# vadimkantorov/deepspeech.pytorch

Hardware: AMD Instinct MI355X
Metric: audio-seconds/sec training, DS2 5x BiGRU-800 bs32, at 1/2/4/8 MI355X (higher is better)
Workload: dtype f32

## Files before the change

### deepspeech.pytorch_amd/csrc/gru_xl.hip

```cpp
#include "rnn_host.h"

#include <algorithm>

namespace ds2 {

#ifndef DS2_XL_ABL
#define DS2_XL_ABL 0
#endif
constexpr bool kAblLoads = (DS2_XL_ABL & 1) != 0;
constexpr bool kAblStores = (DS2_XL_ABL & 2) != 0;
constexpr bool kAblWait = (DS2_XL_ABL & 4) != 0;
constexpr bool kAblFixT = (DS2_XL_ABL & 8) != 0;

constexpr int LB = 8;
constexpr int LU = 32;
constexpr int LW = 4;
constexpr int LT = LW * 64;
constexpr int LSLOTS = 4;
constexpr int LRB = 784;
constexpr int kXlTraceS0 = 100, kXlTraceSteps = 16;

__device__ __forceinline__ bool xl_map(int G, int UBX, int& g, int& ub) {
  g = blockIdx.x & 7;
  ub = blockIdx.x >> 3;
  return g < G && ub < UBX;
}

__device__ __forceinline__ bool xl_group_local(unsigned* xtab, int ub, int UBX, unsigned* err,
                                               unsigned* err_out, int* lds_word, unsigned* mode,
                                               int force_global) {
  const unsigned mine = xcc_id() + 1u;
  if (threadIdx.x == 0) __hip_atomic_store(xtab + ub, mine, __ATOMIC_RELAXED, __HIP_MEMORY_SCOPE_AGENT);
  if ((threadIdx.x >> 6) == 0) {
    const int lane = threadIdx.x & 63;
    unsigned v = mine;
    bool ok = true;
    for (unsigned spins = 0;; ++spins) {
      v = lane < UBX ? __hip_atomic_load(xtab + lane, __ATOMIC_RELAXED, __HIP_MEMORY_SCOPE_AGENT)
                     : mine;
      if (__ballot(v == 0u) == 0ull) break;
      if (spins > g_spin_limit) {
        if (lane == 0) raise_err(err, err_out);
        ok = false;
        break;
      }
      __builtin_amdgcn_s_sleep(1);
    }
    const bool loc = ok && __ballot(v != mine) == 0ull && force_global == 0;
    if (lane == 0) {
      *lds_word = loc ? 1 : 0;
      __hip_atomic_fetch_or(mode, loc ? 1u : 2u, __ATOMIC_RELAXED, __HIP_MEMORY_SCOPE_AGENT);
    }
  }
  __syncthreads();
  return *lds_word != 0;
}

__device__ __forceinline__ void xl_store(u32x4 v, __amdgpu_buffer_rsrc_t rs, int off, bool local) {
  if (local)
    __builtin_amdgcn_raw_buffer_store_b128(v, rs, off, 0, 0);
  else
    __builtin_amdgcn_raw_buffer_store_b128(v, rs, off, 0, kSc1);
}

#define DS2_DPP_MAX(v, ctrl)                                                               \
  v = fmaxf(v, __builtin_bit_cast(float, __builtin_amdgcn_update_dpp(                      \
                   0, __builtin_bit_cast(int, v), ctrl, 0xf, 0xf, true)))
__device__ __forceinline__ float half_wave_max(float v) {
  DS2_DPP_MAX(v, 0xB1);
  DS2_DPP_MAX(v, 0x4E);
  DS2_DPP_MAX(v, 0x141);
  DS2_DPP_MAX(v, 0x140);
  const int b = __builtin_bit_cast(int, v);
  const float r0 = __builtin_bit_cast(float, __builtin_amdgcn_readlane(b, 0));
  const float r1 = __builtin_bit_cast(float, __builtin_amdgcn_readlane(b, 16));
  const float r2 = __builtin_bit_cast(float, __builtin_amdgcn_readlane(b, 32));
  const float r3 = __builtin_bit_cast(float, __builtin_amdgcn_readlane(b, 48));
  return (threadIdx.x & 32) ? fmaxf(r2, r3) : fmaxf(r0, r1);
}
#undef DS2_DPP_MAX

__device__ __forceinline__ bool xl_wave_flags_wait(const unsigned* flags, int count,
                                                   unsigned target, unsigned* err,
                                                   unsigned* err_out) {
  const int lane = threadIdx.x & 63;
  if (count == 0) return true;
  for (unsigned spins = 0;; ++spins) {
    if (spins > g_spin_limit || g_spin_limit == 0) {
      if (lane == 0) raise_err(err, err_out);
      return false;
    }
    const unsigned v = lane < count ? __hip_atomic_load(flags + lane, __ATOMIC_RELAXED,
                                                        __HIP_MEMORY_SCOPE_AGENT)
                                    : target;
    if (__ballot(v < target) == 0ull) return true;
    sleep_units(g_rnn_tune[3]);
  }
}

__device__ __forceinline__ int xl_frag_hi(int m, int k) { return (((k >> 3) << 4) + m) * 8 + (k & 7); }

template <int NPW>
__global__ __launch_bounds__(LT) __attribute__((amdgpu_waves_per_eu(1, 1))) void gru_fwd_xl_kernel(
    int T, int N, int H, int D, int UBX, int BTX, const float* __restrict__ xproj,
    const float* __restrict__ w_f, const float* __restrict__ w_r, const float* __restrict__ b_f,
    const float* __restrict__ b_r, const int* __restrict__ lens, float* __restrict__ h_all,
    float* __restrict__ gates, float* __restrict__ ring, unsigned* __restrict__ xl,
    unsigned* __restrict__ err, unsigned* __restrict__ err_out,
    unsigned long long* __restrict__ stamps, int force_global) {
  constexpr int NCT = 6;
  constexpr int RC = 3 * LU + 1;
  __shared__ float red[LW * 16 * RC];
  __shared__ __attribute__((aligned(16))) _Float16 stg[64 * 8];
  __shared__ float unsc[3 * LU];
  __shared__ __attribute__((aligned(16))) float pin[3 * 256];
  __shared__ __attribute__((aligned(16))) float pout[5 * 256];
  __shared__ int slen[LB];
  __shared__ int sh_local;
  __shared__ int failed;
  __shared__ u32x4 wx[LW * NCT * 2 * 64];
  const int G = D * BTX;
  int g, ub;
  if (!xl_map(G, UBX, g, ub)) return;
  const int d = g / BTX, bt = g - d * BTX;
  const int lane = threadIdx.x & 63;
  const int wave = __builtin_amdgcn_readfirstlane(threadIdx.x >> 6);
  const int p0 = wave * (UBX / LW) + min(wave, UBX % LW);
  const int np = UBX / LW + (wave < UBX % LW ? 1 : 0);
  if (threadIdx.x == 0) failed = 0;
  const bool local =
      xl_group_local(xl + g * 32, ub, UBX, err, err_out, &sh_local, xl + 512 + g, force_global);
  const int slot_floats = G * UBX * 256;
  const __amdgpu_buffer_rsrc_t x_rs =
      __builtin_amdgcn_make_buffer_rsrc(ring, (short)0, LSLOTS * slot_floats * 4, 0x00020000);
  const int grp_off = g * UBX * 256;
  const bool tracing = stamps != nullptr && lane == 0;
  auto trace_at = [&](int s, int p) __attribute__((always_inline)) {
    if (tracing && s >= kXlTraceS0 && s < kXlTraceS0 + kXlTraceSteps)
      stamps[(((int64_t)(s - kXlTraceS0) * gridDim.x + blockIdx.x) * LW + wave) * 6 + p] =
          __builtin_amdgcn_s_memrealtime();
  };

  Duo w[NPW][NCT];
  auto wfr = [&](int p, int ct) __attribute__((always_inline)) {
    if (p < NPW) return w[p < NPW ? p : 0][ct];
    Duo r;
    r.hi = __builtin_bit_cast(f16x8, wx[((wave * NCT + ct) * 2 + 0) * 64 + lane]);
    r.lo = __builtin_bit_cast(f16x8, wx[((wave * NCT + ct) * 2 + 1) * 64 + lane]);
    return r;
  };
  {
    const float* W = d == 0 ? w_f : w_r;
    const int q8 = 8 * (lane >> 4);
    auto frag = [&](int p, int ct, f32x4& a, f32x4& b) __attribute__((always_inline)) {
      const f32x4 z4 = f32x4{0.f, 0.f, 0.f, 0.f};
      if (p < np) {
        const float* r = W + (int64_t)((ct >> 1) * H + LU * ub + 16 * (ct & 1) + (lane & 15)) * H +
                         LU * (p0 + p) + q8;
        a = *reinterpret_cast<const f32x4*>(r);
        b = *reinterpret_cast<const f32x4*>(r + 4);
      } else {
        a = z4;
        b = z4;
      }
    };
    float mx[NCT];
#pragma unroll
    for (int ct = 0; ct < NCT; ++ct) mx[ct] = 0.f;
#pragma unroll
    for (int p = 0; p < NPW + 1; ++p)
#pragma unroll
      for (int ct = 0; ct < NCT; ++ct) {
        f32x4 a, b;
        frag(p, ct, a, b);
#pragma unroll
        for (int i = 0; i < 4; ++i) mx[ct] = fmaxf(mx[ct], fmaxf(fabsf(a[i]), fabsf(b[i])));
      }
#pragma unroll
    for (int ct = 0; ct < NCT; ++ct) {
      mx[ct] = fmaxf(mx[ct], __shfl_xor(mx[ct], 16));
      mx[ct] = fmaxf(mx[ct], __shfl_xor(mx[ct], 32));
      if (lane < 16) red[wave * 96 + ct * 16 + lane] = mx[ct];
    }
    __syncthreads();
    float sc[NCT];
#pragma unroll
    for (int ct = 0; ct < NCT; ++ct) {
      float m = 0.f;
#pragma unroll
      for (int w4 = 0; w4 < LW; ++w4) m = fmaxf(m, red[w4 * 96 + ct * 16 + (lane & 15)]);
      sc[ct] = __builtin_ldexpf(1.f, h3_row_exp(m));
    }
    if (threadIdx.x < 3 * LU) {
      float m = 0.f;
#pragma unroll
      for (int w4 = 0; w4 < LW; ++w4) m = fmaxf(m, red[w4 * 96 + threadIdx.x]);
      unsc[threadIdx.x] = __builtin_ldexpf(1.f, -(h3_row_exp(m) + 14));
    }
    __syncthreads();
    asm volatile("" ::: "memory");
#pragma unroll
    for (int p = 0; p < NPW + 1; ++p)
#pragma unroll
      for (int ct = 0; ct < NCT; ++ct) {
        f32x4 a, b;
        frag(p, ct, a, b);
        const Duo dd = split2h(a, b, sc[ct]);
        if (p < NPW) {
          w[p < NPW ? p : 0][ct] = dd;
        } else {
          wx[((wave * NCT + ct) * 2 + 0) * 64 + lane] = __builtin_bit_cast(u32x4, dd.hi);
          wx[((wave * NCT + ct) * 2 + 1) * 64 + lane] = __builtin_bit_cast(u32x4, dd.lo);
        }
      }
  }
  const float* bh = d == 0 ? b_f : b_r;
  const int m = threadIdx.x >> 5;
  const int u = threadIdx.x & 31;
  const int n = bt * LB + m;
  const int j = ub * LU + u;
  const bool owner = n < N;
  float bias_r = 0.f, bias_z = 0.f, bias_n = 0.f;
  if (owner) {
    bias_r = bh[j];
    bias_z = bh[H + j];
    bias_n = bh[2 * H + j];
  }
  if (threadIdx.x < LB) slen[threadIdx.x] = bt * LB + (int)threadIdx.x < N ? lens[bt * LB + threadIdx.x] : 0;
  __syncthreads();
  const int len = slen[m];
  const float us_r = unsc[u], us_z = unsc[LU + u], us_n = unsc[2 * LU + u];
  settle(bias_r);
  settle(bias_z);
  settle(bias_n);
  const int shi = xl_frag_hi(m, u), slo = shi + 64;
  const bool io = wave != 0;
  const int q = io ? (int)threadIdx.x - 64 : 0;
  const int qm = q / 24, qg = (q % 24) >> 3, q4 = (q & 7) * 4;
  const int qn = bt * LB + qm;
  const bool qv = io && qn < N;
  const int qlen = slen[qm];
  const float* xq = xproj + ((int64_t)qn * D + d) * 3 * H + qg * H + ub * LU + q4;
  const int64_t xstep = (int64_t)N * D * 3 * H;
  const f32x4 z4v = f32x4{0.f, 0.f, 0.f, 0.f};
  auto in_ok = [&](int st) __attribute__((always_inline)) {
    const int tt = d == 0 ? st : T - 1 - st;
    return !kAblLoads && qv && tt < qlen;
  };
  auto load_in = [&](int st) __attribute__((always_inline)) {
    const int tt = d == 0 ? st : T - 1 - st;
    return *reinterpret_cast<const f32x4*>(in_ok(st) ? xq + (kAblFixT ? 0 : tt) * xstep : xproj);
  };
  float* ob[2];
  int64_t ostr[2];
  int osrc[2];
  bool ov[2];
#pragma unroll
  for (int k = 0; k < 2; ++k) {
    const int idx = q + 192 * k;
    const int sm = (idx / 40) & 7, f = (idx % 40) >> 3, o4 = (idx & 7) * 4, sn = bt * LB + sm;
    ov[k] = io && idx < 320 && sn < N && (f == 0 || gates != nullptr);
    osrc[k] = f * 256 + sm * LU + o4;
    if (f == 0) {
      ob[k] = h_all + ((int64_t)sn * D + d) * H + ub * LU + o4;
      ostr[k] = (int64_t)N * D * H;
    } else {
      ob[k] = gates + ((int64_t)sn * D + d) * 4 * H + (f - 1) * H + ub * LU + o4;
      ostr[k] = (int64_t)N * D * 4 * H;
    }
  }
  auto store_out = [&](int st) __attribute__((always_inline)) {
    const int tt = d == 0 ? st : T - 1 - st;
#pragma unroll
    for (int k = 0; k < 2; ++k)
      if (ov[k])
        *reinterpret_cast<f32x4*>(ob[k] + tt * ostr[k]) = *reinterpret_cast<const f32x4*>(pout + osrc[k]);
  };
  f32x4 xin = io ? load_in(0) : z4v;
  float h_own = 0.f;
  for (int s = 0; s < T; ++s) {
    const int t = d == 0 ? s : T - 1 - s;
    f32x4 acc[NCT];
#pragma unroll
    for (int ct = 0; ct < NCT; ++ct) acc[ct] = f32x4{0.f, 0.f, 0.f, 0.f};
    trace_at(s, 0);
    if (io) *reinterpret_cast<f32x4*>(pin + qg * 256 + qm * LU + q4) = in_ok(s) ? xin : z4v;
    if (s > 0) {
      trace_at(s, 1);
      const int base = (((s - 1) % LSLOTS) * slot_floats + grp_off + p0 * 256 + lane * 4) * 4;
      sleep_units(g_rnn_tune[7]);
      u32x4 hv[NPW + 1];
#pragma unroll
      for (int p = 0; p < NPW + 1; ++p)
        hv[p] = __builtin_amdgcn_raw_buffer_load_b128(x_rs, p < np ? base + p * 1024 : 0x7ffffff0, 0, kSc1);
      asm volatile("" ::: "memory");
      __builtin_amdgcn_sched_barrier(0);
      bool bad = false;
#pragma unroll
      for (int p = 0; p < NPW + 1; ++p) {
        if (p < np && !bad) {
          for (unsigned spins = 0;
               !kAblWait && (!wave_ready(__builtin_bit_cast(f32x4, hv[p])) || g_spin_limit == 0);
               ++spins) {
            if (spins > g_spin_limit || g_spin_limit == 0) {
              if (lane == 0) raise_err(err, err_out);
              failed = 1;
              bad = true;
              break;
            }
            sleep_units(g_rnn_tune[0]);
            asm volatile("" ::: "memory");
#pragma unroll
            for (int q = p; q < NPW + 1; ++q)
              if (q < np && (unsigned)(q - p) < g_rnn_tune[6])
                hv[q] = __builtin_amdgcn_raw_buffer_load_b128(x_rs, base + q * 1024, 0, kSc1);
          }
          const f16x8 a = __builtin_bit_cast(f16x8, hv[p]);
#pragma unroll
          for (int ct = 0; ct < NCT; ++ct) {
            const Duo wf = wfr(p, ct);
            acc[ct] = __builtin_amdgcn_mfma_f32_16x16x32_f16(a, wf.lo, acc[ct], 0, 0, 0);
            acc[ct] = __builtin_amdgcn_mfma_f32_16x16x32_f16(a, wf.hi, acc[ct], 0, 0, 0);
          }
        }
      }
      trace_at(s, 2);
    }
    if (io) {
      if (s + 1 < T) xin = load_in(s + 1);
      if (!kAblStores && s > 0) store_out(s - 1);
    }
    trace_at(s, 3);
#pragma unroll
    for (int ct = 0; ct < NCT; ++ct)
#pragma unroll
      for (int i = 0; i < 4; ++i)
        red[(wave * 16 + (lane >> 4) * 4 + i) * RC + ct * 16 + (lane & 15)] = acc[ct][i];
    __syncthreads();
    if (failed) {
      poison_rest(h_all, s, T, d != 0, N, D, n, d, H, j, H, 1, owner);
      return;
    }
    trace_at(s, 4);
    float gh[3];
#pragma unroll
    for (int gt = 0; gt < 3; ++gt) {
      float v = 0.f;
#pragma unroll
      for (int w4 = 0; w4 < LW; ++w4)
        v += red[(w4 * 16 + m) * RC + gt * LU + u] + red[(w4 * 16 + m + 8) * RC + gt * LU + u];
      gh[gt] = v;
    }
    const float xr = pin[m * LU + u], xz = pin[256 + m * LU + u], xn = pin[512 + m * LU + u];
    float hout = 0.f, r = 0.f, z = 0.f, nn = 0.f, ghn = 0.f;
    if (owner && t < len) {
      ghn = gh[2] * us_n + bias_n;
      r = sigmoid_fast(gh[0] * us_r + bias_r + xr);
      z = sigmoid_fast(gh[1] * us_z + bias_z + xz);
      nn = tanh_fast(xn + r * ghn);
      hout = (h_own - nn) * z + nn;
    }
    h_own = owner ? hout : 0.f;
    pout[m * LU + u] = hout;
    pout[256 + m * LU + u] = r;
    pout[512 + m * LU + u] = z;
    pout[768 + m * LU + u] = nn;
    pout[1024 + m * LU + u] = ghn;
    {
      const float v = hout * 16384.f;
      const _Float16 hi = (_Float16)v;
      stg[shi] = hi;
      stg[slo] = (_Float16)(v - (float)hi);
    }
    __syncthreads();
    if (wave == 0) {
      const int toff = (grp_off + ub * 256 + lane * 4) * 4;
      const u32x4 v = desentinel(*reinterpret_cast<const u32x4*>(stg + lane * 8));
      asm volatile("s_waitcnt vmcnt(0)" ::: "memory");
      xl_store(v, x_rs, (s % LSLOTS) * slot_floats * 4 + toff, local);
      xl_store(u32x4{kSentinel, kSentinel, kSentinel, kSentinel}, x_rs,
               ((s + 2) % LSLOTS) * slot_floats * 4 + toff, local);
    }
    trace_at(s, 5);
  }
  __syncthreads();
  if (io && !kAblStores) store_out(T - 1);
}

template <int NPW, bool ROWS>
__global__ __launch_bounds__(LT) __attribute__((amdgpu_waves_per_eu(1, 1))) void gru_bwd_xl_kernel(
    int T, int N, int H, int D, int UBX, int BTX, const float* __restrict__ dy, int dyd,
    const float* __restrict__ w_f, const float* __restrict__ w_r,
    const float* __restrict__ h_all, const float* __restrict__ gates,
    const int* __restrict__ lens, float* __restrict__ dgx, float* __restrict__ dgh,
    float* __restrict__ ring, unsigned* __restrict__ xl, unsigned* __restrict__ err,
    unsigned* __restrict__ err_out, unsigned long long* __restrict__ stamps,
    double* __restrict__ dbp, unsigned* __restrict__ camax, float* __restrict__ rowp,
    int force_global) {
  constexpr int RC = LU + 1;
  constexpr int LWP = 3;
  __shared__ __attribute__((aligned(8))) float red[LW * 16 * RC > 4 * LB * LU * 2 ? LW * 16 * RC : 4 * LB * LU * 2];
  __shared__ __attribute__((aligned(16))) _Float16 stg[3 * 64 * 8];
  __shared__ __attribute__((aligned(16))) float stsc[LB];
  __shared__ float colmx[LW * LU];
  __shared__ __attribute__((aligned(16))) float pin[6 * 256];
  __shared__ __attribute__((aligned(16))) float pout[4 * 256];
  __shared__ int slen[LB];
  __shared__ int sh_local;
  __shared__ int flag;
  __shared__ float rowmx[2 * LB];
  __shared__ u32x4 wx[LW * 6 * 2 * 64];
  const int G = D * BTX;
  int g, ub;
  if (!xl_map(G, UBX, g, ub)) return;
  const int d = g / BTX, bt = g - d * BTX;
  const int lane = threadIdx.x & 63;
  const int wave = __builtin_amdgcn_readfirstlane(threadIdx.x >> 6);
  const int p0 = wave * (UBX / LW) + min(wave, UBX % LW);
  const int np = UBX / LW + (wave < UBX % LW ? 1 : 0);
  const int H3 = 3 * H;
  if (threadIdx.x == 0) flag = 1;
  const int slot_floats = G * UBX * LRB;
  const __amdgpu_buffer_rsrc_t x_rs =
      __builtin_amdgcn_make_buffer_rsrc(ring, (short)0, 2 * slot_floats * 4, 0x00020000);
  const int grp_off = g * UBX * LRB;
  const bool local =
      xl_group_local(xl + g * 32, ub, UBX, err, err_out, &sh_local, xl + 512 + g, force_global);
  unsigned* flags = xl + 256 + g * 32;
  const __amdgpu_buffer_rsrc_t f_rs =
      __builtin_amdgcn_make_buffer_rsrc(xl + 256, (short)0, 8 * 32 * 4, 0x00020000);
  const bool tracing = stamps != nullptr && lane == 0;
  auto trace_at = [&](int s, int p) __attribute__((always_inline)) {
    if (tracing && s >= kXlTraceS0 && s < kXlTraceS0 + kXlTraceSteps)
      stamps[(((int64_t)(s - kXlTraceS0) * gridDim.x + blockIdx.x) * LW + wave) * 6 + p] =
          __builtin_amdgcn_s_memrealtime();
  };

  Duo w[NPW][3][2];
  auto wfr = [&](int p, int gt, int c) __attribute__((always_inline)) {
    if (p < NPW) return w[p < NPW ? p : 0][gt][c];
    Duo r;
    r.hi = __builtin_bit_cast(f16x8, wx[((wave * 6 + gt * 2 + c) * 2 + 0) * 64 + lane]);
    r.lo = __builtin_bit_cast(f16x8, wx[((wave * 6 + gt * 2 + c) * 2 + 1) * 64 + lane]);
    return r;
  };
  float unscale;
  {
    const float* W = d == 0 ? w_f : w_r;
    const int q8 = 8 * (lane >> 4);
    auto col = [&](int p, int gt, int c, f32x4& a, f32x4& b) __attribute__((always_inline)) {
      if (p < np) {
        const float* wc = W + (int64_t)(gt * H + LU * (p0 + p) + q8) * H + LU * ub + 16 * c + (lane & 15);
#pragma unroll
        for (int i = 0; i < 4; ++i) {
          a[i] = wc[(int64_t)i * H];
          b[i] = wc[(int64_t)(i + 4) * H];
        }
      } else {
        a = f32x4{0.f, 0.f, 0.f, 0.f};
        b = a;
      }
    };
    float mx[2] = {0.f, 0.f};
#pragma unroll
    for (int p = 0; p < NPW + 1; ++p)
#pragma unroll
      for (int gt = 0; gt < 3; ++gt)
#pragma unroll
        for (int c = 0; c < 2; ++c) {
          f32x4 a, b;
          col(p, gt, c, a, b);
#pragma unroll
          for (int i = 0; i < 4; ++i) mx[c] = fmaxf(mx[c], fmaxf(fabsf(a[i]), fabsf(b[i])));
        }
#pragma unroll
    for (int c = 0; c < 2; ++c) {
      mx[c] = fmaxf(mx[c], __shfl_xor(mx[c], 16));
      mx[c] = fmaxf(mx[c], __shfl_xor(mx[c], 32));
      if (lane < 16) colmx[wave * LU + 16 * c + lane] = mx[c];
    }
    __syncthreads();
    float sc[2];
#pragma unroll
    for (int c = 0; c < 2; ++c) {
      float m = 0.f;
#pragma unroll
      for (int w4 = 0; w4 < LW; ++w4) m = fmaxf(m, colmx[w4 * LU + 16 * c + (lane & 15)]);
      sc[c] = __builtin_ldexpf(1.f, h3_row_exp(m));
    }
    {
      float m = 0.f;
#pragma unroll
      for (int w4 = 0; w4 < LW; ++w4) m = fmaxf(m, colmx[w4 * LU + (threadIdx.x & 31)]);
      unscale = __builtin_ldexpf(1.f, -h3_row_exp(m));
    }
    asm volatile("" ::: "memory");
#pragma unroll
    for (int p = 0; p < NPW + 1; ++p)
#pragma unroll
      for (int gt = 0; gt < 3; ++gt)
#pragma unroll
        for (int c = 0; c < 2; ++c) {
          f32x4 a, b;
          col(p, gt, c, a, b);
          const Duo dd = split2h(a, b, sc[c]);
          if (p < NPW) {
            w[p < NPW ? p : 0][gt][c] = dd;
          } else {
            wx[((wave * 6 + gt * 2 + c) * 2 + 0) * 64 + lane] = __builtin_bit_cast(u32x4, dd.hi);
            wx[((wave * 6 + gt * 2 + c) * 2 + 1) * 64 + lane] = __builtin_bit_cast(u32x4, dd.lo);
          }
        }
  }
  const int m = threadIdx.x >> 5;
  const int u = threadIdx.x & 31;
  const int n = bt * LB + m;
  const int j = ub * LU + u;
  const bool owner = n < N;
  if (threadIdx.x < LB) slen[threadIdx.x] = bt * LB + (int)threadIdx.x < N ? lens[bt * LB + threadIdx.x] : 0;
  __syncthreads();
  const int len = slen[m];
  const int shi = xl_frag_hi(m, u), slo = shi + 64;
  const bool io = wave != 0;
  const int q = io ? (int)threadIdx.x - 64 : 0;
  const f32x4 z4v = f32x4{0.f, 0.f, 0.f, 0.f};
  const int ostr = N * D * H3;
  struct IoSlot {
    const float* in;
    float* out;
    int f, len, str, pin_at, pout_at;
  };
  auto make_slot = [&](int k) __attribute__((always_inline)) {
    const int idx = q + 192 * k;
    const int sm = idx / 48, f = (idx % 48) >> 3, o4 = (idx & 7) * 4, sn = bt * LB + sm;
    IoSlot r;
    r.f = f;
    r.len = io && sn < N ? slen[sm] : -1;
    if (f == 0) {
      r.in = dy + (sn * dyd + (dyd > 1 ? d : 0)) * H + ub * LU + o4;
      r.str = N * dyd * H;
    } else if (f < 5) {
      r.in = gates + (sn * D + d) * 4 * H + (f - 1) * H + ub * LU + o4;
      r.str = N * D * 4 * H;
    } else {
      r.in = h_all + (sn * D + d) * H + ub * LU + o4;
      r.str = N * D * H;
    }
    r.out = io && sn < N ? (f < 3 ? dgx : dgh) + (sn * D + d) * H3 + (f % 3) * H + ub * LU + o4
                         : nullptr;
    r.pin_at = f * 256 + sm * LU + o4;
    r.pout_at = (f < 3 ? f : (f == 5 ? 3 : f - 3)) * 256 + sm * LU + o4;
    return r;
  };
  const IoSlot sl0 = make_slot(0), sl1 = make_slot(1);
  auto in_ok = [&](int st, const IoSlot sl) __attribute__((always_inline)) {
    const int tt = d == 0 ? T - 1 - st : st;
    const int tr = sl.f == 5 ? (d == 0 ? tt - 1 : tt + 1) : tt;
    return !kAblLoads && tt < sl.len && tr >= 0 && tr < T;
  };
  auto load_in = [&](int st, const IoSlot sl) __attribute__((always_inline)) {
    const int tt = d == 0 ? T - 1 - st : st;
    const int tr = sl.f == 5 ? (d == 0 ? tt - 1 : tt + 1) : tt;
    return *reinterpret_cast<const f32x4*>(sl.in + (in_ok(st, sl) && !kAblFixT ? tr * sl.str : 0));
  };
  auto stage_in = [&](const f32x4 v, const IoSlot sl, int st) __attribute__((always_inline)) {
    *reinterpret_cast<f32x4*>(pin + sl.pin_at) = in_ok(st, sl) ? v : z4v;
  };
  auto store_one = [&](int tt, const IoSlot sl) __attribute__((always_inline)) {
    if (sl.out != nullptr)
      *reinterpret_cast<f32x4*>(sl.out + tt * ostr) = *reinterpret_cast<const f32x4*>(pout + sl.pout_at);
  };
  auto store_out = [&](int st) __attribute__((always_inline)) {
    const int tt = d == 0 ? T - 1 - st : st;
    store_one(tt, sl0);
    store_one(tt, sl1);
  };
  const int rpo = ROWS && wave == 1 && lane < LB && bt * LB + lane < N
                      ? ((bt * LB + lane) * D + d) * UBX + ub
                      : -1;
  const int rpstr = N * D * UBX;
  auto store_rmx = [&](int st) __attribute__((always_inline)) {
    if (!ROWS || wave != 1) return;
    const int tt = d == 0 ? T - 1 - st : st;
    if (rpo >= 0) rowp[rpo + tt * rpstr] = rowmx[(st & 1) * LB + lane];
  };
  f32x4 xin0 = io ? load_in(0, sl0) : z4v, xin1 = io ? load_in(0, sl1) : z4v;
  float dh_prev = 0.f, z_prev = 0.f;
  double sb_r = 0.0, sb_z = 0.0, sb_n = 0.0, sb_hn = 0.0;
  float cm_r = 0.f, cm_z = 0.f, cm_n = 0.f, cm_hn = 0.f;
  const int rsel = ((lane >> 4) & 1) * 16;
  auto io_issue = [&](int st) __attribute__((always_inline)) {
    if (!io) return;
    if (st + 1 < T) {
      xin0 = load_in(st + 1, sl0);
      xin1 = load_in(st + 1, sl1);
    }
    if (!kAblStores && st > 0) store_out(st - 1);
    if (!kAblStores && st > 1) store_rmx(st - 2);
  };
  for (int s = 0; s < T; ++s) {
    const int t = d == 0 ? T - 1 - s : s;
    f32x4 acc[2] = {f32x4{0.f, 0.f, 0.f, 0.f}, f32x4{0.f, 0.f, 0.f, 0.f}};
    trace_at(s, 0);
    if (io) {
      stage_in(xin0, sl0, s);
      stage_in(xin1, sl1, s);
    }
    if (s == 0) io_issue(0);
    if (s > 0) {
      if (!kAblWait && !xl_wave_flags_wait(flags + p0, np, (unsigned)s, err, err_out) && lane == 0)
        flag = 0;
      asm volatile("" ::: "memory");
      trace_at(s, 1);
      const int rb = (((s - 1) & 1) * slot_floats + grp_off + p0 * LRB) * 4;
      u32x4 r0[NPW + 1], r1[NPW + 1], r2[NPW + 1];
      f32x4 rs[NPW + 1];
      auto load_rec = [&](int p) __attribute__((always_inline)) {
        const int base = p < np ? rb + p * LRB * 4 : 0x7ffff000;
        r0[p] = __builtin_amdgcn_raw_buffer_load_b128(x_rs, base + lane * 16, 0, kSc1);
        r1[p] = __builtin_amdgcn_raw_buffer_load_b128(x_rs, base + 1024 + lane * 16, 0, kSc1);
        r2[p] = __builtin_amdgcn_raw_buffer_load_b128(x_rs, base + 2048 + lane * 16, 0, kSc1);
        rs[p] = __builtin_bit_cast(
            f32x4, __builtin_amdgcn_raw_buffer_load_b128(x_rs, base + 3072 + rsel, 0, kSc1));
      };
#pragma unroll
      for (int p = 0; p < LWP && p < NPW + 1; ++p) load_rec(p);
      if (LWP >= NPW + 1) io_issue(s);
      asm volatile("" ::: "memory");
      __builtin_amdgcn_sched_barrier(0);
#pragma unroll
      for (int p = 0; p < NPW + 1; ++p) {
        if (p + LWP < NPW + 1) load_rec(p + LWP);
        if (p + LWP == NPW) io_issue(s);
        if (p < np) {
          const f16x8 ar = __builtin_bit_cast(f16x8, r0[p]);
          const f16x8 az = __builtin_bit_cast(f16x8, r1[p]);
          const f16x8 an = __builtin_bit_cast(f16x8, r2[p]);
#pragma unroll
          for (int c = 0; c < 2; ++c) {
            const f32x4 z4 = f32x4{0.f, 0.f, 0.f, 0.f};
            const Duo w0 = wfr(p, 0, c), w1 = wfr(p, 1, c), w2 = wfr(p, 2, c);
            f32x4 c1 = __builtin_amdgcn_mfma_f32_16x16x32_f16(ar, w0.hi, z4, 0, 0, 0);
            f32x4 c2 = __builtin_amdgcn_mfma_f32_16x16x32_f16(ar, w0.lo, z4, 0, 0, 0);
            c1 = __builtin_amdgcn_mfma_f32_16x16x32_f16(az, w1.hi, c1, 0, 0, 0);
            c2 = __builtin_amdgcn_mfma_f32_16x16x32_f16(az, w1.lo, c2, 0, 0, 0);
            c1 = __builtin_amdgcn_mfma_f32_16x16x32_f16(an, w2.hi, c1, 0, 0, 0);
            c2 = __builtin_amdgcn_mfma_f32_16x16x32_f16(an, w2.lo, c2, 0, 0, 0);
            acc[c] += (c1 + c2) * rs[p];
          }
        }
      }
      trace_at(s, 2);
    }
    trace_at(s, 3);
#pragma unroll
    for (int c = 0; c < 2; ++c)
#pragma unroll
      for (int i = 0; i < 4; ++i)
        red[(wave * 16 + (lane >> 4) * 4 + i) * RC + 16 * c + (lane & 15)] = acc[c][i];
    __syncthreads();
    if (flag == 0) {
      poison_rest(dgx, s, T, d == 0, N, D, n, d, H, j, H3, 3, owner);
      return;
    }
    const float dyv = pin[m * LU + u], g_r = pin[256 + m * LU + u], g_z = pin[512 + m * LU + u];
    const float g_n = pin[768 + m * LU + u], g_hn = pin[1024 + m * LU + u];
    const float hp = pin[1280 + m * LU + u];
    trace_at(s, 4);
    float dar = 0.f, daz = 0.f, dan = 0.f, dghn = 0.f;
    if (owner) {
      float dh = 0.f, zc = 0.f;
      if (t < len) {
        float carry = 0.f;
        if (s > 0) {
          float rec = 0.f;
#pragma unroll
          for (int w4 = 0; w4 < LW; ++w4)
            rec += red[(w4 * 16 + m) * RC + u] + red[(w4 * 16 + m + 8) * RC + u];
          carry = dh_prev * z_prev + rec * unscale;
        }
        dh = dyv + carry;
        zc = g_z;
        dan = dh * (1.f - zc) * (1.f - g_n * g_n);
        daz = dh * (hp - g_n) * zc * (1.f - zc);
        dar = dan * g_hn * g_r * (1.f - g_r);
        dghn = dan * g_r;
      }
      dh_prev = dh;
      z_prev = zc;
      sb_r += dar; sb_z += daz; sb_n += dan; sb_hn += dghn;
      cm_r = fmaxf(cm_r, fabsf(dar));
      cm_z = fmaxf(cm_z, fabsf(daz));
      cm_n = fmaxf(cm_n, fabsf(dan));
      cm_hn = fmaxf(cm_hn, fabsf(dghn));
    }
    pout[m * LU + u] = dar;
    pout[256 + m * LU + u] = daz;
    pout[512 + m * LU + u] = dan;
    pout[768 + m * LU + u] = dghn;
    {
      const float mx = half_wave_max(fmaxf(fmaxf(fabsf(dar), fabsf(daz)), fabsf(dghn)));
      const int e = h3_row_exp(mx);
      const float sc = __builtin_ldexpf(1.f, e);
      const float vr = dar * sc, vz = daz * sc, vn = dghn * sc;
      const _Float16 hr = (_Float16)vr, hz = (_Float16)vz, hn = (_Float16)vn;
      stg[shi] = hr;
      stg[slo] = (_Float16)(vr - (float)hr);
      stg[512 + shi] = hz;
      stg[512 + slo] = (_Float16)(vz - (float)hz);
      stg[1024 + shi] = hn;
      stg[1024 + slo] = (_Float16)(vn - (float)hn);
      if (u == 0) stsc[m] = __builtin_ldexpf(1.f, -e);
    }
    __syncthreads();
    if (wave == 0) {
      const int so = ((s & 1) * slot_floats + grp_off + ub * LRB) * 4;
#pragma unroll
      for (int k = 0; k < 3; ++k)
        xl_store(*reinterpret_cast<const u32x4*>(stg + k * 512 + lane * 8), x_rs,
                 so + k * 1024 + lane * 16, local);
      if (lane < 2) xl_store(*reinterpret_cast<const u32x4*>(stsc + lane * 4), x_rs, so + 3072 + lane * 16, local);
      asm volatile("s_waitcnt vmcnt(0)" ::: "memory");
      if (lane == 0) {
        const unsigned fv = (unsigned)s + 1;
        if (local)
          __builtin_amdgcn_raw_buffer_store_b32(fv, f_rs, (g * 32 + ub) * 4, 0, 0);
        else
          __builtin_amdgcn_raw_buffer_store_b32(fv, f_rs, (g * 32 + ub) * 4, 0, kSc1);
      }
    }
    trace_at(s, 5);
    if (ROWS) {
      const float rm = half_wave_max(fmaxf(fmaxf(fabsf(dar), fabsf(daz)), fabsf(dan)));
      if (u == 0) rowmx[(s & 1) * LB + m] = rm;
    }
  }
  __syncthreads();
  if (io && !kAblStores) store_out(T - 1);
  if (!kAblStores) {
    if (T > 1) store_rmx(T - 2);
    store_rmx(T - 1);
  }
  if (camax != nullptr) {
    __syncthreads();
    red[(0 * LB + m) * LU + u] = cm_r;
    red[(1 * LB + m) * LU + u] = cm_z;
    red[(2 * LB + m) * LU + u] = cm_n;
    red[(3 * LB + m) * LU + u] = cm_hn;
    __syncthreads();
    if (threadIdx.x < 4 * LU) {
      const int gq = threadIdx.x / LU, uu = threadIdx.x - gq * LU;
      float a = 0.f;
#pragma unroll
      for (int mm = 0; mm < LB; ++mm) a = fmaxf(a, red[(gq * LB + mm) * LU + uu]);
      const unsigned bits = __float_as_uint(a);
      const int cl = d * H3 + ub * LU + uu;
      if (bits != 0u) {
        if (gq < 2) {
          atomicMax(camax + cl + gq * H, bits);
          atomicMax(camax + D * H3 + cl + gq * H, bits);
        } else if (gq == 2) {
          atomicMax(camax + cl + 2 * H, bits);
        } else {
          atomicMax(camax + D * H3 + cl + 2 * H, bits);
        }
      }
    }
  }
  if (dbp == nullptr) return;
  double* rd = reinterpret_cast<double*>(red);
  __syncthreads();
  rd[(0 * LB + m) * LU + u] = owner ? sb_r : 0.0;
  rd[(1 * LB + m) * LU + u] = owner ? sb_z : 0.0;
  rd[(2 * LB + m) * LU + u] = owner ? sb_n : 0.0;
  rd[(3 * LB + m) * LU + u] = owner ? sb_hn : 0.0;
  __syncthreads();
  if (threadIdx.x < 4 * LU) {
    const int gq = threadIdx.x / LU, uu = threadIdx.x - gq * LU;
    double a = 0.0;
#pragma unroll
    for (int mm = 0; mm < LB; ++mm) a += rd[(gq * LB + mm) * LU + uu];
    dbp[(((int64_t)bt * D + d) * 4 + gq) * H + ub * LU + uu] = a;
  }
}

__global__ __launch_bounds__(256) void gru_xl_prep_kernel(unsigned* __restrict__ za, size_t na,
                                                          unsigned* __restrict__ zb, size_t nb,
                                                          u32x4* __restrict__ ff, size_t ff16) {
  const size_t i0 = blockIdx.x * (size_t)blockDim.x + threadIdx.x;
  const size_t step = (size_t)gridDim.x * blockDim.x;
  for (size_t i = i0; i < na; i += step) za[i] = 0u;
  for (size_t i = i0; i < nb; i += step) zb[i] = 0u;
  for (size_t i = i0; i < ff16; i += step) ff[i] = u32x4{kSentinel, kSentinel, kSentinel, kSentinel};
}

__global__ __launch_bounds__(256) void gru_xl_row_amax_kernel(const float* __restrict__ rowp,
                                                              int rows, int parts,
                                                              unsigned* __restrict__ out) {
  const int r = (blockIdx.x * 256 + (int)threadIdx.x) >> 3, k = threadIdx.x & 7;
  float m = 0.f;
  if (r < rows)
    for (int i = k; i < parts; i += 8) m = fmaxf(m, rowp[(int64_t)r * parts + i]);
#pragma unroll
  for (int o = 1; o < 8; o <<= 1) m = fmaxf(m, __shfl_xor(m, o));
  if (r < rows && k == 0) out[r] = __float_as_uint(m);
}


static inline bool xl_enabled() { return !env_off("DS2_GRU_XL") && !env_off("DS2_GRU_X6"); }
static inline int xl_force_global() { return env_digit("DS2_GRU_XL") == 2 ? 1 : 0; }

int gru_xl_groups(int n, int h, int num_dirs) {
  if (!xl_enabled() || n < 1 || h < LU || (h % LU) != 0) return 0;
  const int UBX = h / LU, BTX = (n + LB - 1) / LB, G = num_dirs * BTX;
  if (UBX > 32 || G > 8 || (UBX + LW - 1) / LW > 7) return 0;
  return G;
}

int gru_xl_active(int n, int h, int num_dirs) {
  const int G = gru_xl_groups(n, h, num_dirs);
  return G > 0 ? G * (h / LU) : 0;
}

size_t gru_xl_ctr_words() { return 520; }

static const Instance kFwdXl[] = {inst(2, gru_fwd_xl_kernel<1>), inst(4, gru_fwd_xl_kernel<3>),
                                  inst(7, gru_fwd_xl_kernel<6>)};
static const Instance kBwdXl[] = {inst(2, gru_bwd_xl_kernel<1, false>),
                                  inst(4, gru_bwd_xl_kernel<3, false>),
                                  inst(7, gru_bwd_xl_kernel<6, false>)};
static const Instance kBwdXlRows[] = {inst(2, gru_bwd_xl_kernel<1, true>),
                                      inst(4, gru_bwd_xl_kernel<3, true>),
                                      inst(7, gru_bwd_xl_kernel<6, true>)};

size_t gru_xl_ring_bytes(int n, int h, int num_dirs, bool bwd) {
  const size_t UBX = h / LU, G = (size_t)num_dirs * ((n + LB - 1) / LB);
  return bwd ? 2 * G * UBX * LRB * sizeof(float) : LSLOTS * G * UBX * 256 * sizeof(float);
}

static bool xl_prepare(unsigned* ctrs, size_t ctr_bytes, unsigned* zb, size_t nb, float* ring,
                       size_t ff_bytes, hipStream_t st) {
  const size_t na = ctr_bytes / sizeof(unsigned), ff16 = ff_bytes / 16;
  const size_t most = std::max(std::max(na, nb), ff16);
  const unsigned grid = (unsigned)std::min<size_t>(1024, std::max<size_t>(1, (most + 255) / 256));
  hipLaunchKernelGGL(gru_xl_prep_kernel, dim3(grid), dim3(256), 0, st, ctrs, na, zb, nb,
                     reinterpret_cast<u32x4*>(ring), ff16);
  return hipGetLastError() == hipSuccess;
}

bool launch_gru_fwd_xl(RnnShape s, RecFwd a, Handoff ho, hipStream_t st) {
  if (gru_xl_groups(s.n, s.h, s.d) == 0 || env_off("DS2_GRU_H3")) return false;
  apply_spin_limit_env();
  apply_rnn_tune_env();
  int UBX = s.h / LU, BTX = s.BT(LB), FG = xl_force_global();
  const void* fn = pick_instance(kFwdXl, (UBX + LW - 1) / LW);
  if (fn == nullptr) return false;
  if (!xl_prepare(ho.ctrs, ho.ctr_bytes, nullptr, 0, ho.ring,
                  gru_xl_ring_bytes(s.n, s.h, s.d, false), st))
    return false;
  unsigned* xl = ho.err + 1;
  void* args[] = {&s.t, &s.n, &s.h, &s.d, &UBX, &BTX, &a.xproj, &a.w_hh_f, &a.w_hh_r, &a.b_hh_f,
                  &a.b_hh_r, &a.lens, &a.h_all, &a.gates, &ho.ring, &xl, &ho.err, &ho.err_out,
                  &ho.stamps, &FG};
  return rnn_launch(fn, dim3(8 * UBX), dim3(LT), args, ho.lds_pad, st) == hipSuccess;
}

bool launch_gru_bwd_xl(RnnShape s, RecBwd a, Handoff ho, hipStream_t st) {
  if (gru_xl_groups(s.n, s.h, s.d) == 0 || env_off("DS2_GRU_H3_BWD")) return false;
  apply_spin_limit_env();
  apply_rnn_tune_env();
  int UBX = s.h / LU, BTX = s.BT(LB), FG = xl_force_global();
  const int need = (UBX + LW - 1) / LW;
  const void* fn = a.rowp != nullptr ? pick_instance(kBwdXlRows, need) : pick_instance(kBwdXl, need);
  if (fn == nullptr) return false;
  if (!xl_prepare(ho.ctrs, ho.ctr_bytes, a.camax,
                  a.camax != nullptr ? (size_t)2 * s.d * 3 * s.h : 0, nullptr, 0, st))
    return false;
  unsigned* xl = ho.err + 1;
  void* args[] = {&s.t, &s.n, &s.h, &s.d, &UBX, &BTX, &a.dy, &a.dy_dirs, &a.w_hh_f, &a.w_hh_r,
                  &a.state, &a.gates, &a.lens, &a.dgx, &a.dgh, &ho.ring, &xl, &ho.err,
                  &ho.err_out, &ho.stamps, &a.dbp, &a.camax, &a.rowp, &FG};
  return rnn_launch(fn, dim3(8 * UBX), dim3(LT), args, ho.lds_pad, st) == hipSuccess;
}

size_t gru_xl_rowp_bytes(int t_max, int n, int h, int num_dirs) {
  return (size_t)t_max * n * num_dirs * (h / LU) * sizeof(float);
}

void launch_gru_xl_row_amax(int t_max, int n, int h, int num_dirs, const float* rowp,
                            unsigned* out, hipStream_t st) {
  const int rows = t_max * n;
  hipLaunchKernelGGL(gru_xl_row_amax_kernel, dim3((rows * 8 + 255) / 256), dim3(256), 0, st, rowp,
                     rows, num_dirs * (h / LU), out);
}

}
```

Before: 9377.

## Pin GRU XL recurrent weights in AGPRs and issue MFMA chains via inline asm

The persistent GRU forward and backward XL kernels now keep most recurrent weight fragments in accumulator registers (AGPRs), with only the first one or two panels left in VGPRs. The per-step MFMA sequences are written as hand-scheduled inline asm blocks with explicit s_nop hazard padding. Tracing is made a compile-time template parameter, and the error and poison state moves into a shared-memory struct, so the hot loop carries fewer live registers and branches. The aim is to relieve VGPR pressure and cut instruction overhead on the latency-bound recurrent step. In exchange, the hand-written hazard nops may over- or under-pad, and the manual asm constrains the compiler's scheduling.

```diff
diff --git a/deepspeech.pytorch_amd/csrc/gru_xl.hip b/deepspeech.pytorch_amd/csrc/gru_xl.hip
--- a/deepspeech.pytorch_amd/csrc/gru_xl.hip
+++ b/deepspeech.pytorch_amd/csrc/gru_xl.hip
@@ -24,6 +24,28 @@
   g = blockIdx.x & 7;
   ub = blockIdx.x >> 3;
   return g < G && ub < UBX;
+}
+
+typedef __attribute__((address_space(1))) unsigned xl_gu32;
+typedef __attribute__((address_space(1))) float xl_gf32;
+struct XlCold {
+  xl_gu32 *err, *err_out;
+  xl_gf32* out;
+  int N, D, H;
+  int n0, j0;
+};
+
+__device__ __forceinline__ void xl_raise(const XlCold& c) {
+  xl_gu32 *e = c.err, *eo = c.err_out;
+  __hip_atomic_fetch_or(e, 1u, __ATOMIC_RELAXED, __HIP_MEMORY_SCOPE_AGENT);
+  if (eo != nullptr) __hip_atomic_fetch_or(eo, 1u, __ATOMIC_RELAXED, __HIP_MEMORY_SCOPE_AGENT);
+}
+
+__device__ __forceinline__ void xl_poison(const XlCold& c, int s, int T, bool rev, int d,
+                                          int width_h, int groups) {
+  const int n = c.n0 + (int)(threadIdx.x >> 5);
+  poison_rest((float*)c.out, s, T, rev, c.N, c.D, n, d, c.H, c.j0 + (int)(threadIdx.x & 31),
+              width_h * c.H, groups, n < c.N);
 }
 
 __device__ __forceinline__ bool xl_group_local(unsigned* xtab, int ub, int UBX, unsigned* err,
@@ -81,13 +103,12 @@
 #undef DS2_DPP_MAX
 
 __device__ __forceinline__ bool xl_wave_flags_wait(const unsigned* flags, int count,
-                                                   unsigned target, unsigned* err,
-                                                   unsigned* err_out) {
+                                                   unsigned target, const XlCold& cold) {
   const int lane = threadIdx.x & 63;
   if (count == 0) return true;
   for (unsigned spins = 0;; ++spins) {
     if (spins > g_spin_limit || g_spin_limit == 0) {
-      if (lane == 0) raise_err(err, err_out);
+      if (lane == 0) xl_raise(cold);
       return false;
     }
     const unsigned v = lane < count ? __hip_atomic_load(flags + lane, __ATOMIC_RELAXED,
@@ -98,9 +119,65 @@
   }
 }
 
+constexpr int kXlVgprW = 2, kXlVgprWBwd = 1;
+__device__ __forceinline__ u32x4 xl_agpr(u32x4 v) {
+  u32x4 r;
+  asm volatile("" : "=a"(r) : "0"(v));
+  return r;
+}
+__device__ __forceinline__ void xl_mfma_settle(f32x4 (&c)[6]) {
+  asm volatile("s_nop 15\n\ts_nop 7"
+               : "+v"(c[0]), "+v"(c[1]), "+v"(c[2]), "+v"(c[3]), "+v"(c[4]), "+v"(c[5]));
+}
+#define DS2_XL_FWD_TILE(WC)                                                                  \
+  asm volatile(                                                                              \
+      "s_nop 1\n\t"                                                                          \
+      "v_mfma_f32_16x16x32_f16 %0, %6, %7, %0\n\tv_mfma_f32_16x16x32_f16 %1, %6, %8, %1\n\t"  \
+      "v_mfma_f32_16x16x32_f16 %2, %6, %9, %2\n\tv_mfma_f32_16x16x32_f16 %3, %6, %10, %3\n\t" \
+      "v_mfma_f32_16x16x32_f16 %4, %6, %11, %4\n\tv_mfma_f32_16x16x32_f16 %5, %6, %12, %5\n\t" \
+      "v_mfma_f32_16x16x32_f16 %0, %6, %13, %0\n\tv_mfma_f32_16x16x32_f16 %1, %6, %14, %1\n\t" \
+      "v_mfma_f32_16x16x32_f16 %2, %6, %15, %2\n\tv_mfma_f32_16x16x32_f16 %3, %6, %16, %3\n\t" \
+      "v_mfma_f32_16x16x32_f16 %4, %6, %17, %4\n\tv_mfma_f32_16x16x32_f16 %5, %6, %18, %5"      \
+      : "+v"(c[0]), "+v"(c[1]), "+v"(c[2]), "+v"(c[3]), "+v"(c[4]), "+v"(c[5])               \
+      : "v"(a), WC(lo[0]), WC(lo[1]), WC(lo[2]), WC(lo[3]), WC(lo[4]), WC(lo[5]), WC(hi[0]), \
+        WC(hi[1]), WC(hi[2]), WC(hi[3]), WC(hi[4]), WC(hi[5]))
+template <bool AG>
+__device__ __forceinline__ void xl_fwd_tile(f32x4 (&c)[6], u32x4 a, const u32x4 (&lo)[6],
+                                            const u32x4 (&hi)[6]) {
+  if constexpr (AG)
+    DS2_XL_FWD_TILE("a");
+  else
+    DS2_XL_FWD_TILE("v");
+}
+#undef DS2_XL_FWD_TILE
+
+#define DS2_XL_BWD_REC(WC)                                                                    \
+  asm volatile(                                                                               \
+      "s_nop 1\n\t"                                                                           \
+      "v_mfma_f32_16x16x32_f16 %0, %4, %7, 0\n\tv_mfma_f32_16x16x32_f16 %1, %4, %8, 0\n\t"     \
+      "v_mfma_f32_16x16x32_f16 %2, %4, %9, 0\n\tv_mfma_f32_16x16x32_f16 %3, %4, %10, 0\n\t"    \
+      "v_mfma_f32_16x16x32_f16 %0, %5, %11, %0\n\tv_mfma_f32_16x16x32_f16 %1, %5, %12, %1\n\t" \
+      "v_mfma_f32_16x16x32_f16 %2, %5, %13, %2\n\tv_mfma_f32_16x16x32_f16 %3, %5, %14, %3\n\t" \
+      "v_mfma_f32_16x16x32_f16 %0, %6, %15, %0\n\tv_mfma_f32_16x16x32_f16 %1, %6, %16, %1\n\t" \
+      "v_mfma_f32_16x16x32_f16 %2, %6, %17, %2\n\tv_mfma_f32_16x16x32_f16 %3, %6, %18, %3\n\t" \
+      "s_nop 9"                                                                               \
+      : "=&v"(c[0]), "=&v"(c[1]), "=&v"(c[2]), "=&v"(c[3])                                    \
+      : "v"(ar), "v"(az), "v"(an), WC(w[0][0][0]), WC(w[0][0][1]), WC(w[0][1][0]),            \
+        WC(w[0][1][1]), WC(w[1][0][0]), WC(w[1][0][1]), WC(w[1][1][0]), WC(w[1][1][1]),       \
+        WC(w[2][0][0]), WC(w[2][0][1]), WC(w[2][1][0]), WC(w[2][1][1]))
+template <bool AG>
+__device__ __forceinline__ void xl_bwd_rec(f32x4 (&c)[4], u32x4 ar, u32x4 az, u32x4 an,
+                                           const u32x4 (&w)[3][2][2]) {
+  if constexpr (AG)
+    DS2_XL_BWD_REC("a");
+  else
+    DS2_XL_BWD_REC("v");
+}
+#undef DS2_XL_BWD_REC
+
 __device__ __forceinline__ int xl_frag_hi(int m, int k) { return (((k >> 3) << 4) + m) * 8 + (k & 7); }
 
-template <int NPW>
+template <int NPW, bool TRACE>
 __global__ __launch_bounds__(LT) __attribute__((amdgpu_waves_per_eu(1, 1))) void gru_fwd_xl_kernel(
     int T, int N, int H, int D, int UBX, int BTX, const float* __restrict__ xproj,
     const float* __restrict__ w_f, const float* __restrict__ w_r, const float* __restrict__ b_f,
@@ -118,6 +195,7 @@
   __shared__ int slen[LB];
   __shared__ int sh_local;
   __shared__ int failed;
+  __shared__ XlCold cold;
   __shared__ u32x4 wx[LW * NCT * 2 * 64];
   const int G = D * BTX;
   int g, ub;
@@ -127,28 +205,24 @@
   const int wave = __builtin_amdgcn_readfirstlane(threadIdx.x >> 6);
   const int p0 = wave * (UBX / LW) + min(wave, UBX % LW);
   const int np = UBX / LW + (wave < UBX % LW ? 1 : 0);
-  if (threadIdx.x == 0) failed = 0;
+  if (threadIdx.x == 0) {
+    failed = 0;
+    cold = XlCold{(xl_gu32*)err, (xl_gu32*)err_out, (xl_gf32*)h_all, N, D, H, bt * LB, ub * LU};
+  }
   const bool local =
       xl_group_local(xl + g * 32, ub, UBX, err, err_out, &sh_local, xl + 512 + g, force_global);
   const int slot_floats = G * UBX * 256;
   const __amdgpu_buffer_rsrc_t x_rs =
       __builtin_amdgcn_make_buffer_rsrc(ring, (short)0, LSLOTS * slot_floats * 4, 0x00020000);
   const int grp_off = g * UBX * 256;
-  const bool tracing = stamps != nullptr && lane == 0;
   auto trace_at = [&](int s, int p) __attribute__((always_inline)) {
-    if (tracing && s >= kXlTraceS0 && s < kXlTraceS0 + kXlTraceSteps)
-      stamps[(((int64_t)(s - kXlTraceS0) * gridDim.x + blockIdx.x) * LW + wave) * 6 + p] =
-          __builtin_amdgcn_s_memrealtime();
-  };
-
-  Duo w[NPW][NCT];
-  auto wfr = [&](int p, int ct) __attribute__((always_inline)) {
-    if (p < NPW) return w[p < NPW ? p : 0][ct];
-    Duo r;
-    r.hi = __builtin_bit_cast(f16x8, wx[((wave * NCT + ct) * 2 + 0) * 64 + lane]);
-    r.lo = __builtin_bit_cast(f16x8, wx[((wave * NCT + ct) * 2 + 1) * 64 + lane]);
-    return r;
-  };
+    if constexpr (TRACE)
+      if (stamps != nullptr && lane == 0 && s >= kXlTraceS0 && s < kXlTraceS0 + kXlTraceSteps)
+        stamps[(((int64_t)(s - kXlTraceS0) * gridDim.x + blockIdx.x) * LW + wave) * 6 + p] =
+            __builtin_amdgcn_s_memrealtime();
+  };
+
+  u32x4 whi[NPW][NCT], wlo[NPW][NCT];
   {
     const float* W = d == 0 ? w_f : w_r;
     const int q8 = 8 * (lane >> 4);
@@ -206,11 +280,13 @@
         f32x4 a, b;
         frag(p, ct, a, b);
         const Duo dd = split2h(a, b, sc[ct]);
+        const u32x4 dh = __builtin_bit_cast(u32x4, dd.hi), dl = __builtin_bit_cast(u32x4, dd.lo);
         if (p < NPW) {
-          w[p < NPW ? p : 0][ct] = dd;
+          whi[p < NPW ? p : 0][ct] = p < kXlVgprW ? dh : xl_agpr(dh);
+          wlo[p < NPW ? p : 0][ct] = p < kXlVgprW ? dl : xl_agpr(dl);
         } else {
-          wx[((wave * NCT + ct) * 2 + 0) * 64 + lane] = __builtin_bit_cast(u32x4, dd.hi);
-          wx[((wave * NCT + ct) * 2 + 1) * 64 + lane] = __builtin_bit_cast(u32x4, dd.lo);
+          wx[((wave * NCT + ct) * 2 + 0) * 64 + lane] = dh;
+          wx[((wave * NCT + ct) * 2 + 1) * 64 + lane] = dl;
         }
       }
   }
@@ -290,20 +366,23 @@
       const int base = (((s - 1) % LSLOTS) * slot_floats + grp_off + p0 * 256 + lane * 4) * 4;
       sleep_units(g_rnn_tune[7]);
       u32x4 hv[NPW + 1];
+      int npl = np;
+      asm volatile("" : "+s"(npl));
 #pragma unroll
       for (int p = 0; p < NPW + 1; ++p)
-        hv[p] = __builtin_amdgcn_raw_buffer_load_b128(x_rs, p < np ? base + p * 1024 : 0x7ffffff0, 0, kSc1);
+        hv[p] = __builtin_amdgcn_raw_buffer_load_b128(x_rs, p < npl ? base + p * 1024 : 0x7ffffff0, 0, kSc1);
       asm volatile("" ::: "memory");
       __builtin_amdgcn_sched_barrier(0);
       bool bad = false;
 #pragma unroll
       for (int p = 0; p < NPW + 1; ++p) {
-        if (p < np && !bad) {
+        if (p >= npl) break;
+        if (!bad) {
           for (unsigned spins = 0;
                !kAblWait && (!wave_ready(__builtin_bit_cast(f32x4, hv[p])) || g_spin_limit == 0);
                ++spins) {
             if (spins > g_spin_limit || g_spin_limit == 0) {
-              if (lane == 0) raise_err(err, err_out);
+              if (lane == 0) xl_raise(cold);
               failed = 1;
               bad = true;
               break;
@@ -312,18 +391,25 @@
             asm volatile("" ::: "memory");
 #pragma unroll
             for (int q = p; q < NPW + 1; ++q)
-              if (q < np && (unsigned)(q - p) < g_rnn_tune[6])
+              if (q < npl && (unsigned)(q - p) < g_rnn_tune[6])
                 hv[q] = __builtin_amdgcn_raw_buffer_load_b128(x_rs, base + q * 1024, 0, kSc1);
           }
-          const f16x8 a = __builtin_bit_cast(f16x8, hv[p]);
+        }
+        if (p < kXlVgprW && p < NPW) {
+          xl_fwd_tile<false>(acc, hv[p], wlo[p < NPW ? p : 0], whi[p < NPW ? p : 0]);
+        } else if (p < NPW) {
+          xl_fwd_tile<true>(acc, hv[p], wlo[p < NPW ? p : 0], whi[p < NPW ? p : 0]);
+        } else {
+          u32x4 xh[NCT], xw[NCT];
 #pragma unroll
           for (int ct = 0; ct < NCT; ++ct) {
-            const Duo wf = wfr(p, ct);
-            acc[ct] = __builtin_amdgcn_mfma_f32_16x16x32_f16(a, wf.lo, acc[ct], 0, 0, 0);
-            acc[ct] = __builtin_amdgcn_mfma_f32_16x16x32_f16(a, wf.hi, acc[ct], 0, 0, 0);
+            xh[ct] = wx[((wave * NCT + ct) * 2 + 0) * 64 + lane];
+            xw[ct] = wx[((wave * NCT + ct) * 2 + 1) * 64 + lane];
           }
+          xl_fwd_tile<false>(acc, hv[p], xw, xh);
         }
       }
+      xl_mfma_settle(acc);
       trace_at(s, 2);
     }
     if (io) {
@@ -338,7 +424,7 @@
         red[(wave * 16 + (lane >> 4) * 4 + i) * RC + ct * 16 + (lane & 15)] = acc[ct][i];
     __syncthreads();
     if (failed) {
-      poison_rest(h_all, s, T, d != 0, N, D, n, d, H, j, H, 1, owner);
+      xl_poison(cold, s, T, d != 0, d, 1, 1);
       return;
     }
     trace_at(s, 4);
@@ -387,7 +473,7 @@
   if (io && !kAblStores) store_out(T - 1);
 }
 
-template <int NPW, bool ROWS>
+template <int NPW, bool ROWS, bool TRACE>
 __global__ __launch_bounds__(LT) __attribute__((amdgpu_waves_per_eu(1, 1))) void gru_bwd_xl_kernel(
     int T, int N, int H, int D, int UBX, int BTX, const float* __restrict__ dy, int dyd,
     const float* __restrict__ w_f, const float* __restrict__ w_r,
@@ -408,6 +494,7 @@
   __shared__ int slen[LB];
   __shared__ int sh_local;
   __shared__ int flag;
+  __shared__ XlCold cold;
   __shared__ float rowmx[2 * LB];
   __shared__ u32x4 wx[LW * 6 * 2 * 64];
   const int G = D * BTX;
@@ -419,7 +506,10 @@
   const int p0 = wave * (UBX / LW) + min(wave, UBX % LW);
   const int np = UBX / LW + (wave < UBX % LW ? 1 : 0);
   const int H3 = 3 * H;
-  if (threadIdx.x == 0) flag = 1;
+  if (threadIdx.x == 0) {
+    flag = 1;
+    cold = XlCold{(xl_gu32*)err, (xl_gu32*)err_out, (xl_gf32*)dgx, N, D, H, bt * LB, ub * LU};
+  }
   const int slot_floats = G * UBX * LRB;
   const __amdgpu_buffer_rsrc_t x_rs =
       __builtin_amdgcn_make_buffer_rsrc(ring, (short)0, 2 * slot_floats * 4, 0x00020000);
@@ -429,21 +519,14 @@
   unsigned* flags = xl + 256 + g * 32;
   const __amdgpu_buffer_rsrc_t f_rs =
       __builtin_amdgcn_make_buffer_rsrc(xl + 256, (short)0, 8 * 32 * 4, 0x00020000);
-  const bool tracing = stamps != nullptr && lane == 0;
   auto trace_at = [&](int s, int p) __attribute__((always_inline)) {
-    if (tracing && s >= kXlTraceS0 && s < kXlTraceS0 + kXlTraceSteps)
-      stamps[(((int64_t)(s - kXlTraceS0) * gridDim.x + blockIdx.x) * LW + wave) * 6 + p] =
-          __builtin_amdgcn_s_memrealtime();
-  };
-
-  Duo w[NPW][3][2];
-  auto wfr = [&](int p, int gt, int c) __attribute__((always_inline)) {
-    if (p < NPW) return w[p < NPW ? p : 0][gt][c];
-    Duo r;
-    r.hi = __builtin_bit_cast(f16x8, wx[((wave * 6 + gt * 2 + c) * 2 + 0) * 64 + lane]);
-    r.lo = __builtin_bit_cast(f16x8, wx[((wave * 6 + gt * 2 + c) * 2 + 1) * 64 + lane]);
-    return r;
-  };
+    if constexpr (TRACE)
+      if (stamps != nullptr && lane == 0 && s >= kXlTraceS0 && s < kXlTraceS0 + kXlTraceSteps)
+        stamps[(((int64_t)(s - kXlTraceS0) * gridDim.x + blockIdx.x) * LW + wave) * 6 + p] =
+            __builtin_amdgcn_s_memrealtime();
+  };
+
+  u32x4 w[NPW][3][2][2];
   float unscale;
   {
     const float* W = d == 0 ? w_f : w_r;
@@ -504,18 +587,19 @@
           f32x4 a, b;
           col(p, gt, c, a, b);
           const Duo dd = split2h(a, b, sc[c]);
+          const u32x4 dh = __builtin_bit_cast(u32x4, dd.hi), dl = __builtin_bit_cast(u32x4, dd.lo);
           if (p < NPW) {
-            w[p < NPW ? p : 0][gt][c] = dd;
+            w[p < NPW ? p : 0][gt][c][0] = p < kXlVgprWBwd ? dh : xl_agpr(dh);
+            w[p < NPW ? p : 0][gt][c][1] = p < kXlVgprWBwd ? dl : xl_agpr(dl);
           } else {
-            wx[((wave * 6 + gt * 2 + c) * 2 + 0) * 64 + lane] = __builtin_bit_cast(u32x4, dd.hi);
-            wx[((wave * 6 + gt * 2 + c) * 2 + 1) * 64 + lane] = __builtin_bit_cast(u32x4, dd.lo);
+            wx[((wave * 6 + gt * 2 + c) * 2 + 0) * 64 + lane] = dh;
+            wx[((wave * 6 + gt * 2 + c) * 2 + 1) * 64 + lane] = dl;
           }
         }
   }
   const int m = threadIdx.x >> 5;
   const int u = threadIdx.x & 31;
   const int n = bt * LB + m;
-  const int j = ub * LU + u;
   const bool owner = n < N;
   if (threadIdx.x < LB) slen[threadIdx.x] = bt * LB + (int)threadIdx.x < N ? lens[bt * LB + threadIdx.x] : 0;
   __syncthreads();
@@ -608,7 +692,9 @@
     }
     if (s == 0) io_issue(0);
     if (s > 0) {
-      if (!kAblWait && !xl_wave_flags_wait(flags + p0, np, (unsigned)s, err, err_out) && lane == 0)
+      int npl = np;
+      asm volatile("" : "+s"(npl));
+      if (!kAblWait && !xl_wave_flags_wait(flags + p0, npl, (unsigned)s, cold) && lane == 0)
         flag = 0;
       asm volatile("" ::: "memory");
       trace_at(s, 1);
@@ -616,7 +702,7 @@
       u32x4 r0[NPW + 1], r1[NPW + 1], r2[NPW + 1];
       f32x4 rs[NPW + 1];
       auto load_rec = [&](int p) __attribute__((always_inline)) {
-        const int base = p < np ? rb + p * LRB * 4 : 0x7ffff000;
+        const int base = p < npl ? rb + p * LRB * 4 : 0x7ffff000;
         r0[p] = __builtin_amdgcn_raw_buffer_load_b128(x_rs, base + lane * 16, 0, kSc1);
         r1[p] = __builtin_amdgcn_raw_buffer_load_b128(x_rs, base + 1024 + lane * 16, 0, kSc1);
         r2[p] = __builtin_amdgcn_raw_buffer_load_b128(x_rs, base + 2048 + lane * 16, 0, kSc1);
@@ -632,22 +718,21 @@
       for (int p = 0; p < NPW + 1; ++p) {
         if (p + LWP < NPW + 1) load_rec(p + LWP);
         if (p + LWP == NPW) io_issue(s);
-        if (p < np) {
-          const f16x8 ar = __builtin_bit_cast(f16x8, r0[p]);
-          const f16x8 az = __builtin_bit_cast(f16x8, r1[p]);
-          const f16x8 an = __builtin_bit_cast(f16x8, r2[p]);
-#pragma unroll
-          for (int c = 0; c < 2; ++c) {
-            const f32x4 z4 = f32x4{0.f, 0.f, 0.f, 0.f};
-            const Duo w0 = wfr(p, 0, c), w1 = wfr(p, 1, c), w2 = wfr(p, 2, c);
-            f32x4 c1 = __builtin_amdgcn_mfma_f32_16x16x32_f16(ar, w0.hi, z4, 0, 0, 0);
-            f32x4 c2 = __builtin_amdgcn_mfma_f32_16x16x32_f16(ar, w0.lo, z4, 0, 0, 0);
-            c1 = __builtin_amdgcn_mfma_f32_16x16x32_f16(az, w1.hi, c1, 0, 0, 0);
-            c2 = __builtin_amdgcn_mfma_f32_16x16x32_f16(az, w1.lo, c2, 0, 0, 0);
-            c1 = __builtin_amdgcn_mfma_f32_16x16x32_f16(an, w2.hi, c1, 0, 0, 0);
-            c2 = __builtin_amdgcn_mfma_f32_16x16x32_f16(an, w2.lo, c2, 0, 0, 0);
-            acc[c] += (c1 + c2) * rs[p];
+        if (p < npl) {
+          f32x4 cc[4];
+          if (p < kXlVgprWBwd && p < NPW) {
+            xl_bwd_rec<false>(cc, r0[p], r1[p], r2[p], w[p < NPW ? p : 0]);
+          } else if (p < NPW) {
+            xl_bwd_rec<true>(cc, r0[p], r1[p], r2[p], w[p < NPW ? p : 0]);
+          } else {
+            u32x4 xw[3][2][2];
+#pragma unroll
+            for (int k = 0; k < 12; ++k)
+              xw[k >> 2][(k >> 1) & 1][k & 1] = wx[(wave * 12 + k) * 64 + lane];
+            xl_bwd_rec<false>(cc, r0[p], r1[p], r2[p], xw);
           }
+          acc[0] += (cc[0] + cc[1]) * rs[p];
+          acc[1] += (cc[2] + cc[3]) * rs[p];
         }
       }
       trace_at(s, 2);
@@ -660,7 +745,7 @@
         red[(wave * 16 + (lane >> 4) * 4 + i) * RC + 16 * c + (lane & 15)] = acc[c][i];
     __syncthreads();
     if (flag == 0) {
-      poison_rest(dgx, s, T, d == 0, N, D, n, d, H, j, H3, 3, owner);
+      xl_poison(cold, s, T, d == 0, d, 3, 3);
       return;
     }
     const float dyv = pin[m * LU + u], g_r = pin[256 + m * LU + u], g_z = pin[512 + m * LU + u];
@@ -824,14 +909,15 @@
 
 size_t gru_xl_ctr_words() { return 520; }
 
-static const Instance kFwdXl[] = {inst(2, gru_fwd_xl_kernel<1>), inst(4, gru_fwd_xl_kernel<3>),
-                                  inst(7, gru_fwd_xl_kernel<6>)};
-static const Instance kBwdXl[] = {inst(2, gru_bwd_xl_kernel<1, false>),
-                                  inst(4, gru_bwd_xl_kernel<3, false>),
-                                  inst(7, gru_bwd_xl_kernel<6, false>)};
-static const Instance kBwdXlRows[] = {inst(2, gru_bwd_xl_kernel<1, true>),
-                                      inst(4, gru_bwd_xl_kernel<3, true>),
-                                      inst(7, gru_bwd_xl_kernel<6, true>)};
+#define DS2_XL_TABLE(K, ...) \
+  {inst(2, K<1, __VA_ARGS__>), inst(4, K<3, __VA_ARGS__>), inst(7, K<6, __VA_ARGS__>)}
+static const Instance kFwdXl[2][3] = {DS2_XL_TABLE(gru_fwd_xl_kernel, false),
+                                      DS2_XL_TABLE(gru_fwd_xl_kernel, true)};
+static const Instance kBwdXl[2][3] = {DS2_XL_TABLE(gru_bwd_xl_kernel, false, false),
+                                      DS2_XL_TABLE(gru_bwd_xl_kernel, false, true)};
+static const Instance kBwdXlRows[2][3] = {DS2_XL_TABLE(gru_bwd_xl_kernel, true, false),
+                                          DS2_XL_TABLE(gru_bwd_xl_kernel, true, true)};
+#undef DS2_XL_TABLE
 
 size_t gru_xl_ring_bytes(int n, int h, int num_dirs, bool bwd) {
   const size_t UBX = h / LU, G = (size_t)num_dirs * ((n + LB - 1) / LB);
@@ -853,7 +939,7 @@
   apply_spin_limit_env();
   apply_rnn_tune_env();
   int UBX = s.h / LU, BTX = s.BT(LB), FG = xl_force_global();
-  const void* fn = pick_instance(kFwdXl, (UBX + LW - 1) / LW);
+  const void* fn = pick_instance(kFwdXl[ho.stamps != nullptr], (UBX + LW - 1) / LW);
   if (fn == nullptr) return false;
   if (!xl_prepare(ho.ctrs, ho.ctr_bytes, nullptr, 0, ho.ring,
                   gru_xl_ring_bytes(s.n, s.h, s.d, false), st))
@@ -871,7 +957,9 @@
   apply_rnn_tune_env();
   int UBX = s.h / LU, BTX = s.BT(LB), FG = xl_force_global();
   const int need = (UBX + LW - 1) / LW;
-  const void* fn = a.rowp != nullptr ? pick_instance(kBwdXlRows, need) : pick_instance(kBwdXl, need);
+  const int tr = ho.stamps != nullptr;
+  const void* fn =
+      a.rowp != nullptr ? pick_instance(kBwdXlRows[tr], need) : pick_instance(kBwdXl[tr], need);
   if (fn == nullptr) return false;
   if (!xl_prepare(ho.ctrs, ho.ctr_bytes, a.camax,
                   a.camax != nullptr ? (size_t)2 * s.d * 3 * s.h : 0, nullptr, 0, st))
```

Result: faster. 10410 (median of 6 runs) (+11.1%).
